# see--/speech_recognition

Measured on AMD Instinct MI355X. Metric: 1s 16kHz clips/sec training throughput, higher is better.
Workload: dtype f32; 1 GPU; configs[1]: 12-class conv_1d_time_sliced_with_attention, batch 1024/GPU synthetic 16000-sample fp32 clips, sampler+augment+STFT/mel(80,60)+raw fwd/bwd+RMSprop; global_batch=1024, parallelism=dp1, clip_bank=65536

## Files before the change

### include/kws_hip.h

```cpp
#ifndef KWS_HIP_H_
#define KWS_HIP_H_

#include <stdint.h>

#ifdef __cplusplus
extern "C" {
#endif
#if defined(__GNUC__) || defined(__clang__)
#pragma GCC visibility push(default)
#endif

#define KWS_OK 0
#define KWS_E_INVALID (-1)
#define KWS_E_HIP (-2)
#define KWS_E_WORKSPACE (-3)

#define KWS_ABI_VERSION 5

int kws_abi_version(void);
const char* kws_last_error(void);
int kws_device_name(char* buf, int cap);

int kws_stream_create(int cls, void** stream);
int kws_stream_destroy(void* stream);
// ... 72 lines not shown
int kws_comm_destroy(kws_comm_t* comm);
int kws_allreduce_grads(kws_comm_t* comm, float* grads, int64_t n, void* stream);

int kws_head32to12(const float* p_in, int C_in, const int32_t* map, int C_out, float* p_out,
                   int B, void* stream);

typedef struct kws_stft_plan kws_stft_plan_t;
int kws_stft_plan_create(int frame_len, int frame_step, int fft_len, int n_mel, int n_out,
                         const float* window, const float* mel, const float* dct,
                         float log_offset, float log_floor, kws_stft_plan_t** plan);
int kws_stft_plan_destroy(kws_stft_plan_t* plan);
int kws_stft_num_frames(const kws_stft_plan_t* plan, int L);
int kws_stft_mel_f32(const kws_stft_plan_t* plan, const float* x, int B, int L, float* out,
                     int out_kind, void* stream);

int kws_absmax_batch_f32(const float* const* in, const int64_t* n, unsigned* slots, int count, void* stream);
int kws_dwconv_fwd_amax_f32(const float* y, const float* bn, const float* w, float* z, int B, int L_in, int L_out,
                            int C, int stride, int pad_l, unsigned* amax, void* stream);
int kws_dwconv_bwd_bn_amax_f32(const float* dz, const float* y, const float* bn, const float* w, const float* coef,
                               float* dy, float* part, int pass, int B, int L_in, int L_out, int C, int stride, int pad_l,
                               unsigned* amax, void* stream);
int kws_bn_bwd_apply_amax(float* g, const float* y, const float* bn, const float* gamma, const float* coef, int64_t rows,
                          int C, unsigned* amax, void* stream);
int kws_f16x2_split_batch(const float* const* in, void* const* out, const int* rows, const int* cols,
                          const int* transpose, const unsigned* const* slots, int count, void* stream);
int kws_gemm_nn_f16x2_supported(int64_t M, int K, int N);
int kws_gemm_tn_f16x2_supported(int64_t M, int K, int N);
int kws_gemm_nn_f16x2_stats_rows(int64_t M);
int kws_gemm_nn_f16x2_f32(const float* A, const void* Bp, float* C, int64_t M, int K, int N,
                          const unsigned* a_slots, const unsigned* b_slots, float* stats_part, void* stream);
int64_t kws_gemm_tn_f16x2_workspace_floats(int64_t M, int K, int N);
int kws_gemm_tn_f16x2_f32(const float* Z, const float* G, float* dW, int64_t M, int K, int N,
                          const unsigned* z_slots, const unsigned* g_slots, float* workspace, void* stream);

int kws_gemm_num_row_tiles(int64_t M);
int kws_gemm_nn_stats_rows(int64_t M, int K, int N);
int kws_gemm_gather_stats_rows(int64_t M);
int kws_gemm_nn_f32(const float* A, const float* W, float* C, int64_t M, int K, int N,
                    float* stats_part, void* stream);
typedef struct {
  int L_out;
  int cin;
  int taps;
  int stride_t;
  int stride_j;
  int base_off;
// ... 211 lines not shown
  int kind;
  int num_classes;
  int filter_mult;
  int input_size;
  int spectrogram_length;
  int num_features;
} kws_net_config_t;
typedef struct {
  char name[64];
  int64_t offset;
  int64_t size;
  int ndim;
  int64_t shape[4];
  int is_state;
  float l2;
  int fan_in, fan_out;
  float init;
} kws_tensor_info_t;

int kws_net_create(const kws_net_config_t* cfg, kws_net_t** net);
int kws_net_destroy(kws_net_t* net);
int kws_net_get_gemm_mode(const kws_net_t* net);
int kws_net_set_gemm_mode(kws_net_t* net, int mode);
int64_t kws_net_num_params(const kws_net_t* net);
int64_t kws_net_num_state(const kws_net_t* net);
int kws_net_num_tensors(const kws_net_t* net);
int kws_net_tensor_info(const kws_net_t* net, int idx, kws_tensor_info_t* info);
int64_t kws_net_workspace_bytes(const kws_net_t* net, int max_batch, int training);
int kws_net_debug_view(const kws_net_t* net, int batch, int training, int what, int index,
                       int64_t* offset_floats, int64_t* count);
int kws_net_predict(const kws_net_t* net, const float* params, const float* state, const float* x,
                    int B, float* probs, void* workspace, int64_t workspace_bytes, void* stream);
int kws_net_train_fwd_bwd(const kws_net_t* net, const float* params, float* state, const float* x,
                          const float* y_onehot, int B, float* grads, float* probs, float* metrics,
                          uint64_t seed, uint32_t step, int64_t row_offset, int loss_batch,
                          void* workspace, int64_t workspace_bytes, void* stream);

int kws_net_num_blocks(const kws_net_t* net);
int64_t kws_net_grad_ready_offset(const kws_net_t* net, int split_block);
int kws_net_train_fwd_bwd_part(const kws_net_t* net, const float* params, float* state, const float* x,
                               const float* y_onehot, int B, float* grads, float* probs, float* metrics,
                               uint64_t seed, uint32_t step, int64_t row_offset, int loss_batch,
                               void* workspace, int64_t workspace_bytes, int part, int split_block,
                               void* stream);

#if defined(__GNUC__) || defined(__clang__)
// ... 7 lines not shown
```

### speech_recognition_amd/_lib.py

```python
import ctypes
import os

_HERE = os.path.dirname(os.path.abspath(__file__))
LIB_PATH = os.environ.get("KWS_LIB_PATH") or os.path.join(_HERE, "libkws_hip.so")

ABI_VERSION = 5

KWS_NET_TS_ATTENTION = 1
KWS_NET_LOG_MFCC = 2
KWS_NET_STEFFE = 3
KWS_NET_RESIDUAL = 4
KWS_NET_MFCC_AND_RAW = 5
KWS_NET_CONV_1D_FAST = 6
KWS_NET_CONV_1D_SPEC = 7
KWS_NET_CONV_1D_TIME_STACKED = 8
KWS_NET_CONV_1D_HEAVY = 9
KWS_NET_CONV_1D_GRU = 10
KWS_NET_CONV_1D_MULTI_TIME_SLICED = 11
KWS_NET_CONV_1D_SIMPLE = 12
KWS_NET_XCEPTION_ATTENTION = 13
KWS_NET_INCEPTION_D1 = 14
KWS_NET_CONV_2D_MOBILE = 15
KWS_NET_CONV_2D_FAST = 16
KWS_NET_CONV_1D_TIME_SLICED = 17
# ... 108 lines not shown
    "kws_allreduce_grads": (_I, [_P, _P, _I64, _P]),
    "kws_stretch_plan_create": (_I, [_I, ctypes.c_double, ctypes.POINTER(_P)]),
    "kws_stretch_plan_destroy": (_I, [_P]),
    "kws_stretch_out_samples": (_I, [_P]),
    "kws_time_stretch_f32": (_I, [_P, _P, _F, _P, _I, _I, _I, _P]),
    "kws_time_stretch_i16": (_I, [_P, _P, _P, _I, _I, _I, _P]),
    "kws_stft_plan_create": (_I, [_I, _I, _I, _I, _I, _P, _P, _P, _F, _F, ctypes.POINTER(_P)]),
    "kws_stft_plan_destroy": (_I, [_P]),
    "kws_stft_num_frames": (_I, [_P, _I]),
    "kws_stft_mel_f32": (_I, [_P, _P, _I, _I, _P, _I, _P]),
    "kws_gemm_num_row_tiles": (_I, [_I64]),
    "kws_gemm_nn_stats_rows": (_I, [_I64, _I, _I]),
    "kws_gemm_gather_stats_rows": (_I, [_I64]),
    "kws_gemm_nn_f32": (_I, [_P, _P, _P, _I64, _I, _I, _P, _P]),
    "kws_net_get_gemm_mode": (_I, [_P]),
    "kws_net_set_gemm_mode": (_I, [_P, _I]),
    "kws_gemm_nn_f16x2_supported": (_I, [_I64, _I, _I]),
    "kws_gemm_tn_f16x2_supported": (_I, [_I64, _I, _I]),
    "kws_gemm_nn_f16x2_stats_rows": (_I, [_I64]),
    "kws_absmax_batch_f32": (_I, [_P, _P, _P, _I, _P]),
    "kws_dwconv_fwd_amax_f32": (_I, [_P, _P, _P, _P, _I, _I, _I, _I, _I, _I, _P, _P]),
    "kws_dwconv_bwd_bn_amax_f32": (_I, [_P, _P, _P, _P, _P, _P, _P, _I, _I, _I, _I, _I, _I, _I, _P, _P]),
    "kws_bn_bwd_apply_amax": (_I, [_P, _P, _P, _P, _P, _I64, _I, _P, _P]),
    "kws_f16x2_split_batch": (_I, [_P, _P, _P, _P, _P, _P, _I, _P]),
    "kws_gemm_nn_f16x2_f32": (_I, [_P, _P, _P, _I64, _I, _I, _P, _P, _P, _P]),
    "kws_gemm_tn_f16x2_workspace_floats": (_I64, [_I64, _I, _I]),
    "kws_gemm_tn_f16x2_f32": (_I, [_P, _P, _P, _I64, _I, _I, _P, _P, _P, _P]),
    "kws_gemm_gather_f32": (_I, [_P, ctypes.POINTER(GatherDesc), _P, _P, _I, _I, _P, _P]),
    "kws_gemm_tn_workspace_floats": (_I64, [_I64, _I, _I]),
    "kws_gemm_tn_f32": (_I, [_P, _P, _P, _I64, _I, _I, _P, _P]),
    "kws_gemm_tn_gather_f32": (_I, [_P, ctypes.POINTER(GatherDesc), _P, _P, _I, _I, _P, _P]),
    "kws_gconv_stats_rows": (_I, [ctypes.POINTER(GconvDesc)]),
    "kws_gconv_fwd_f32": (_I, [_P, _P, _I, _P, _P, _P, ctypes.POINTER(GconvDesc), _P]),
    "kws_gconv_dgrad_f32": (_I, [_P, _P, _P, ctypes.POINTER(GconvDesc), _P]),
    "kws_gconv_wgrad_workspace_floats": (_I64, [ctypes.POINTER(GconvDesc)]),
    "kws_gconv_wgrad_f32": (_I, [_P, _P, _I, _P, _P, _P, ctypes.POINTER(GconvDesc), _P]),
    "kws_pool3s2_out_len": (_I, [_I]),
    "kws_pool3s2_fwd_f32": (_I, [_P, _P, _P, _I, _I, _I, _P]),
    "kws_pool3s2_bwd_part_rows": (_I, [_I, _I, _I]),
    "kws_pool3s2_bwd_part_floats": (_I64, [_I, _I, _I]),
    "kws_pool3s2_bwd_f32": (_I, [_P, _P, _P, _P, _P, _I, _I, _I, _P]),
    "kws_pool3s2_same_out_len": (_I, [_I]),
    "kws_pool3s2_same_fwd_f32": (_I, [_P, _P, _P, _I, _I, _I, _P]),
    "kws_pool3s2_same_bwd_part_rows": (_I, [_I, _I, _I]),
    "kws_pool3s2_same_bwd_part_floats": (_I64, [_I, _I, _I]),
    "kws_pool3s2_same_bwd_f32": (_I, [_P, _P, _P, _P, _P, _I, _I, _I, _P]),
# ... 197 lines not shown
```

### speech_recognition_amd/csrc/dw_bwd_body.h

```cpp
#pragma once
#include "internal.h"

namespace kws_dw {

#ifndef KWS_DW_NT
#define KWS_DW_NT 1
#endif
typedef float dw_v4f __attribute__((ext_vector_type(4)));
__device__ __forceinline__ float4 ld4_stream(const float* p) {
  if (KWS_DW_NT & 2) {
    const dw_v4f v = __builtin_nontemporal_load(reinterpret_cast<const dw_v4f*>(p));
    return make_float4(v.x, v.y, v.z, v.w);
  }
  return *reinterpret_cast<const float4*>(p);
}
__device__ __forceinline__ void st4_stream(float* p, float4 o) {
  if (KWS_DW_NT & 1) {
    dw_v4f v = {o.x, o.y, o.z, o.w};
    __builtin_nontemporal_store(v, reinterpret_cast<dw_v4f*>(p));
    return;
  }
  *reinterpret_cast<float4*>(p) = o;
}

// ... 2 lines not shown
#endif
constexpr int TT = KWS_DW_TT;

__device__ __forceinline__ float4 f4_fma(float4 a, float4 b, float4 c) {
  return make_float4(fmaf(a.x, b.x, c.x), fmaf(a.y, b.y, c.y), fmaf(a.z, b.z, c.z), fmaf(a.w, b.w, c.w));
}
__device__ __forceinline__ float4 f4_mul(float4 a, float4 b) {
  return make_float4(a.x * b.x, a.y * b.y, a.z * b.z, a.w * b.w);
}
__device__ __forceinline__ float4 f4_zero() { return make_float4(0.f, 0.f, 0.f, 0.f); }

#ifndef DW_BWD_THREADS
#define DW_BWD_THREADS 512
#endif
#ifndef DW_BWD_HT
#define DW_BWD_HT 8
#endif
#ifndef DW_BWD2_THREADS
#define DW_BWD2_THREADS 512
#endif
#ifndef DW_BWD_PARTS
#define DW_BWD_PARTS 256
#endif

struct BwdArgs {
  const float* dz; const float* y; const float* bn; const float* w; const float* coef;
  float* g; float* part;
  int B, Lin, Lout, C, pad_l, nchunks, R, Cb;
  unsigned* amax;
  int add_stride = 0, add_len = 0;
};
constexpr int bwd_smem_floats(int mode, int threads) { return mode == 2 ? 4 : 5 * threads * 4; }

template <int S, bool HAS_BN, int MODE, bool GUARD, bool ADDS = false>
__device__ __forceinline__ void bwd_body(const BwdArgs& p, float* const red, const int bid, const int nblk, const int by) {
  const float* __restrict__ dz = p.dz;
  const float* __restrict__ y = p.y;
  const float* __restrict__ bn = p.bn;
  const float* __restrict__ w = p.w;
  const float* __restrict__ coef = p.coef;
  float* __restrict__ g = p.g;
  float* __restrict__ part = p.part;
  const int B = p.B, Lin = p.Lin, Lout = p.Lout, C = p.C, pad_l = p.pad_l, nchunks = p.nchunks, R = p.R, Cb = p.Cb;
  constexpr int RSTRIDE = (MODE == 2 ? 4 : DW_BWD_THREADS * 4);
  float gmax = 0.f;
  const int C4 = Cb >> 2;
  const int tid = threadIdx.x;
  const bool live = !GUARD || tid < R * C4;
  const int r = live ? tid / C4 : 0, c4 = live ? tid - r * C4 : 0;
  const int c = by * Cb + c4 * 4;
  float4 sg = f4_zero(), sgx = f4_zero(), sw0 = f4_zero(), sw1 = f4_zero(), sw2 = f4_zero();
  float4 sc = f4_zero(), sh = f4_zero(), mean = f4_zero(), rstd = f4_zero();
  if (HAS_BN) {
    sc = *reinterpret_cast<const float4*>(bn + c);
    sh = *reinterpret_cast<const float4*>(bn + C + c);
    mean = *reinterpret_cast<const float4*>(bn + 2 * C + c);
    rstd = *reinterpret_cast<const float4*>(bn + 3 * C + c);
  }
  const float4 w0 = *reinterpret_cast<const float4*>(w + c);
  const float4 w1 = *reinterpret_cast<const float4*>(w + C + c);
  const float4 w2 = *reinterpret_cast<const float4*>(w + 2 * C + c);
  float4 c1 = f4_zero(), c2 = f4_zero();
  if (MODE == 2) {
    c1 = *reinterpret_cast<const float4*>(coef + c);
    c2 = *reinterpret_cast<const float4*>(coef + C + c);
  }
  for (int64_t ub = bid; ub * R < (int64_t)B * nchunks; ub += nblk) {
    const int64_t unit = ub * R + r;
    const int64_t b = unit / nchunks;
    const int chunk = (int)(unit - b * nchunks);
    if (b >= B || !live) continue;
    const float* yb = y + b * (int64_t)Lin * C + c;
    float* gb = g + b * (int64_t)Lin * C + c;
    const float* dzb = dz + b * (int64_t)Lout * C + c;
    const int u0 = chunk * TT;
    constexpr int HT = DW_BWD_HT;
    constexpr int ND = S == 1 ? HT + 2 : HT / 2 + 2;
    const bool podd = (pad_l & 1) != 0;
#pragma unroll
    for (int h = 0; h < TT / HT; ++h) {
      const int ub = u0 + h * HT;
      if (ub >= Lin) break;
      float4 yv[HT], D[ND];
#pragma unroll
      for (int i = 0; i < HT; ++i) yv[i] = ld4_stream(yb + (int64_t)(ub + i < Lin ? ub + i : ub) * C);
      const int t_lo = S == 1 ? ub + pad_l - 2 : ((ub + pad_l) >> 1) - 1;
#pragma unroll
      for (int j = 0; j < ND; ++j) {
        const int t = t_lo + j;
        D[j] = ld4_stream(dzb + (int64_t)(t < 0 ? 0 : (t < Lout ? t : Lout - 1)) * C);
      }
// ... 115 lines not shown
```

### speech_recognition_amd/csrc/dwconv.hip

```cpp
#include "dw_bwd_body.h"

namespace {
using namespace kws_dw;

#ifndef DW_FWD_GRID
#define DW_FWD_GRID 4096
#endif

template <int S, bool HAS_BN>
__global__ __launch_bounds__(256) void dwconv_fwd_kernel(const float* __restrict__ y, const float* __restrict__ bn,
                                                         const float* __restrict__ w, float* __restrict__ z,
                                                         int B, int Lin, int Lout, int C, int pad_l, int nchunks,
                                                         unsigned* amax) {
  const int C4 = C >> 2;
  float zmax = 0.f;
  const int64_t total = (int64_t)B * nchunks * C4;
  for (int64_t id = (int64_t)blockIdx.x * 256 + threadIdx.x; id < total; id += (int64_t)gridDim.x * 256) {
    const int c4 = (int)(id % C4);
    const int64_t rest = id / C4;
    const int chunk = (int)(rest % nchunks);
    const int64_t b = rest / nchunks;
    const int c = c4 * 4;
    float4 sc = f4_zero(), sh = f4_zero();
    if (HAS_BN) {
      sc = *reinterpret_cast<const float4*>(bn + c);
      sh = *reinterpret_cast<const float4*>(bn + C + c);
    }
    const float4 w0 = *reinterpret_cast<const float4*>(w + c);
    const float4 w1 = *reinterpret_cast<const float4*>(w + C + c);
    const float4 w2 = *reinterpret_cast<const float4*>(w + 2 * C + c);
    const float* yb = y + b * (int64_t)Lin * C + c;
    float* zb = z + b * (int64_t)Lout * C + c;
    constexpr int NL = S == 1 ? TT + 2 : 2 * TT + 1;
    const int t0 = chunk * TT;
    const int u_lo = S * t0 - pad_l;
    float4 av[NL];
#pragma unroll
    for (int k = 0; k < NL; ++k) {
      const int u = u_lo + k;
      av[k] = ld4_stream(yb + (int64_t)(u >= 0 && u < Lin ? u : 0) * C);
// ... 23 lines not shown
  }
  if (amax) kws_absmax_commit(amax, zmax);
}

#ifndef KWS_DW_BWD2_MINW
#define KWS_DW_BWD2_MINW 1
#endif
#ifndef KWS_DW_BWD1_MINW
#define KWS_DW_BWD1_MINW 1
#endif
template <int S, bool HAS_BN, int MODE, bool ADDS = false>
__global__ __launch_bounds__(MODE == 2 ? DW_BWD2_THREADS : DW_BWD_THREADS, MODE == 2 ? KWS_DW_BWD2_MINW : KWS_DW_BWD1_MINW) void dwconv_bwd_kernel(BwdArgs p) {
  __shared__ float red[bwd_smem_floats(MODE, DW_BWD_THREADS)];
  bwd_body<S, HAS_BN, MODE, false, ADDS>(p, red, (int)blockIdx.x, (int)gridDim.x, (int)blockIdx.y);
}

}


namespace {
template <int MODE>
int launch_dw_bwd(const float* dz, const float* y, const float* bn, const float* w, const float* coef, float* g,
                  float* part, int B, int L_in, int L_out, int C, int stride, int pad_l, hipStream_t st,
                  unsigned* amax = nullptr, int add_stride = 0, int add_len = 0) {
  const BwdGeom ge = bwd_geom(B, L_in, C, MODE != 2);
  KWS_REQUIRE(ge.grid < 0x7FFFFFFF, "dwconv_bwd: grid too large");
  dim3 gr((unsigned)ge.grid, (unsigned)ge.ny), b((unsigned)ge.block);
  BwdArgs a;
  a.dz = dz; a.y = y; a.bn = bn; a.w = w; a.coef = coef; a.g = g; a.part = part;
  a.B = B; a.Lin = L_in; a.Lout = L_out; a.C = C; a.pad_l = pad_l; a.nchunks = ge.nchunks; a.R = ge.R; a.Cb = ge.Cb; a.amax = amax;
  a.add_stride = add_stride; a.add_len = add_len;
  if (MODE == 0 && add_stride > 1) {
    if (stride == 1) hipLaunchKernelGGL((dwconv_bwd_kernel<1, false, MODE, true>), gr, b, 0, st, a);
    else hipLaunchKernelGGL((dwconv_bwd_kernel<2, false, MODE, true>), gr, b, 0, st, a);
    KWS_LAUNCH_CHECK("dwconv_bwd_kernel");
    return KWS_OK;
  }
  if (stride == 1) {
    if (bn) hipLaunchKernelGGL((dwconv_bwd_kernel<1, true, MODE>), gr, b, 0, st, a);
    else hipLaunchKernelGGL((dwconv_bwd_kernel<1, false, MODE>), gr, b, 0, st, a);
  } else {
    if (bn) hipLaunchKernelGGL((dwconv_bwd_kernel<2, true, MODE>), gr, b, 0, st, a);
    else hipLaunchKernelGGL((dwconv_bwd_kernel<2, false, MODE>), gr, b, 0, st, a);
  }
  KWS_LAUNCH_CHECK("dwconv_bwd_kernel");
  return KWS_OK;
}
}

extern "C" {

int kws_dwconv_fwd_f32(const float* y, const float* bn, const float* w, float* z, int B, int L_in, int L_out,
                       int C, int stride, int pad_l, void* stream) {
  return kws_dwconv_fwd_amax_f32(y, bn, w, z, B, L_in, L_out, C, stride, pad_l, nullptr, (hipStream_t)stream);
}

int kws_dwconv_fwd_amax_f32(const float* y, const float* bn, const float* w, float* z, int B, int L_in, int L_out,
                            int C, int stride, int pad_l, unsigned* amax, void* stream_) {
  hipStream_t stream = (hipStream_t)stream_;
  KWS_REQUIRE(y && w && z, "dwconv_fwd: NULL pointer");
  KWS_REQUIRE(B > 0 && L_in > 0 && L_out > 0 && C > 0 && C % 4 == 0, "dwconv_fwd: bad shape B=%d L=%d->%d C=%d",
              B, L_in, L_out, C);
  KWS_REQUIRE(stride == 1 || stride == 2, "dwconv_fwd: stride %d unsupported", stride);
  KWS_REQUIRE(pad_l >= 0 && stride * (L_out - 1) + 2 - pad_l < L_in + 2, "dwconv_fwd: geometry reads past padding");
  const int nchunks = ceil_div(L_out, TT);
  const int64_t threads = (int64_t)B * nchunks * (C / 4);
  int64_t grid = ceil_div64(threads, 256);
  if (grid > DW_FWD_GRID) grid = DW_FWD_GRID;
  dim3 g((unsigned)grid), b(256);
  hipStream_t st = (hipStream_t)stream;
  KwsProfScope prof("dwconv_fwd", 6.0 * B * L_out * C, 4.0 * ((double)B * L_in * C + (double)B * L_out * C), st);
  if (stride == 1) {
    if (bn) hipLaunchKernelGGL((dwconv_fwd_kernel<1, true>), g, b, 0, st, y, bn, w, z, B, L_in, L_out, C, pad_l, nchunks, amax);
    else hipLaunchKernelGGL((dwconv_fwd_kernel<1, false>), g, b, 0, st, y, bn, w, z, B, L_in, L_out, C, pad_l, nchunks, amax);
  } else {
    if (bn) hipLaunchKernelGGL((dwconv_fwd_kernel<2, true>), g, b, 0, st, y, bn, w, z, B, L_in, L_out, C, pad_l, nchunks, amax);
    else hipLaunchKernelGGL((dwconv_fwd_kernel<2, false>), g, b, 0, st, y, bn, w, z, B, L_in, L_out, C, pad_l, nchunks, amax);
  }
  KWS_LAUNCH_CHECK("dwconv_fwd_kernel");
  return KWS_OK;
}

int64_t kws_dwconv_bwd_part_floats(int B, int L_in, int C) {
  if (B <= 0 || L_in <= 0 || !bwd_geom_ok(C)) return 0;
  const BwdGeom g = bwd_geom(B, L_in, C);
  return g.grid * 5 * C;
}

int kws_dwconv_bwd_f32(const float* dz, const float* y, const float* bn, const float* w, float* g, float* part,
                       int B, int L_in, int L_out, int C, int stride, int pad_l, void* stream) {
  KWS_REQUIRE(dz && y && w && g && part, "dwconv_bwd: NULL pointer");
  KWS_REQUIRE(B > 0 && L_in > 0 && L_out > 0 && bwd_geom_ok(C),
              "dwconv_bwd: bad shape B=%d L=%d->%d C=%d", B, L_in, L_out, C);
  KWS_REQUIRE(stride == 1 || stride == 2, "dwconv_bwd: stride %d unsupported", stride);
  hipStream_t st = (hipStream_t)stream;
  KwsProfScope prof("dwconv_bwd", 12.0 * B * L_in * C, 4.0 * (2.0 * B * L_in * C + (double)B * L_out * C), st);
  return launch_dw_bwd<0>(dz, y, bn, w, nullptr, g, part, B, L_in, L_out, C, stride, pad_l, st);
}

int kws_dwconv_bwd_acc_f32(const float* dz, const float* y, const float* w, const float* add, float* g, float* part, int B,
// ... 4 lines not shown
  KwsProfScope prof("dwconv_bwd", 13.0 * B * L_in * C, 4.0 * (3.0 * B * L_in * C + (double)B * L_out * C), st);
  return launch_dw_bwd<0>(dz, y, nullptr, w, add, g, part, B, L_in, L_out, C, stride, pad_l, st);
}

int kws_dwconv_bwd_acc_strided_f32(const float* dz, const float* y, const float* w, const float* add, int add_stride, int add_len,
                                   float* g, float* part, int B, int L_in, int L_out, int C, int stride, int pad_l, hipStream_t st) {
  KWS_REQUIRE(dz && y && w && add && g && part && add != g, "dwconv_bwd_acc_strided: bad pointers");
  KWS_REQUIRE(B > 0 && L_in > 0 && L_out > 0 && bwd_geom_ok(C) && (stride == 1 || stride == 2) && add_stride >= 2 && add_len > 0 &&
                  (int64_t)(add_len - 1) * add_stride < L_in,
              "dwconv_bwd_acc_strided: bad shape B=%d L=%d->%d C=%d stride=%d add %d x %d", B, L_in, L_out, C, stride, add_len, add_stride);
  KwsProfScope prof("dwconv_bwd", 13.0 * B * L_in * C, 4.0 * (2.0 * B * L_in * C + (double)B * L_out * C + (double)B * add_len * C), st);
  return launch_dw_bwd<0>(dz, y, nullptr, w, add, g, part, B, L_in, L_out, C, stride, pad_l, st, nullptr, add_stride, add_len);
}

int kws_dwconv_bwd_bn_f32(const float* dz, const float* y, const float* bn, const float* w, const float* coef,
                          float* dy, float* part, int pass, int B, int L_in, int L_out, int C, int stride, int pad_l,
                          void* stream) {
  return kws_dwconv_bwd_bn_amax_f32(dz, y, bn, w, coef, dy, part, pass, B, L_in, L_out, C, stride, pad_l, nullptr,
                                    (hipStream_t)stream);
}

int kws_dwconv_bwd_bn_amax_f32(const float* dz, const float* y, const float* bn, const float* w, const float* coef,
                               float* dy, float* part, int pass, int B, int L_in, int L_out, int C, int stride, int pad_l,
                               unsigned* amax, void* stream_) {
  hipStream_t stream = (hipStream_t)stream_;
  KWS_REQUIRE(dz && y && bn && w, "dwconv_bwd_bn: NULL pointer");
  KWS_REQUIRE(pass == 1 ? part != nullptr : (pass == 2 && coef != nullptr && dy != nullptr),
              "dwconv_bwd_bn: pass %d needs %s", pass, pass == 1 ? "part" : "coef and dy");
  KWS_REQUIRE(B > 0 && L_in > 0 && L_out > 0 && bwd_geom_ok(C),
              "dwconv_bwd_bn: bad shape B=%d L=%d->%d C=%d", B, L_in, L_out, C);
  KWS_REQUIRE(stride == 1 || stride == 2, "dwconv_bwd_bn: stride %d unsupported", stride);
  hipStream_t st = (hipStream_t)stream;
  KwsProfScope prof("dwconv_bwd", 12.0 * B * L_in * C,
                    4.0 * ((pass == 2 ? 2.0 : 1.0) * B * L_in * C + (double)B * L_out * C), st);
  if (pass == 1) return launch_dw_bwd<1>(dz, y, bn, w, nullptr, nullptr, part, B, L_in, L_out, C, stride, pad_l, st);
  return launch_dw_bwd<2>(dz, y, bn, w, coef, dy, nullptr, B, L_in, L_out, C, stride, pad_l, st, amax);
}

}
```

### speech_recognition_amd/csrc/net.hip

```cpp
#include "net_internal.h"
#include <math.h>
#include <stdlib.h>

int64_t kws_net_add_tensor(kws_net* n, const std::string& name, std::vector<int64_t> shape, bool is_state, float l2,
                           int fan_in, int fan_out, float init) {
  kws_tensor_info_t t;
  memset(&t, 0, sizeof(t));
  snprintf(t.name, sizeof(t.name), "%s", name.c_str());
  int64_t size = 1;
  t.ndim = (int)shape.size();
  for (int i = 0; i < t.ndim; ++i) {
    t.shape[i] = shape[i];
    size *= shape[i];
  }
  t.size = size;
  t.is_state = is_state ? 1 : 0;
  t.l2 = l2;
  t.fan_in = fan_in;
  t.fan_out = fan_out;
  t.init = init;
  int64_t& cursor = is_state ? n->n_state : n->n_params;
  t.offset = cursor;
  cursor += (size + 3) / 4 * 4;
  n->tensors.push_back(t);
// ... 485 lines not shown
}

int kws_net_debug_view(const kws_net_t* net, int batch, int training, int what, int index, int64_t* offset_floats,
                       int64_t* count) {
  KWS_REQUIRE(net && offset_floats && count && batch > 0, "net_debug_view: bad arguments");
  return net->program->debug_view(batch, training, what, index, offset_floats, count);
}

int kws_net_predict(const kws_net_t* net, const float* params, const float* state, const float* x, int B,
                    float* probs, void* workspace, int64_t workspace_bytes, void* stream) {
  KWS_REQUIRE(net && params && state && x && probs && workspace && B > 0, "net_predict: bad arguments");
  return net->program->predict(params, state, x, B, probs, (float*)workspace, workspace_bytes, (hipStream_t)stream);
}

extern "C" int kws_net_get_gemm_mode(const kws_net_t* net) { return net ? net->gemm_mode.load(std::memory_order_relaxed) : 0; }
extern "C" int kws_net_set_gemm_mode(kws_net_t* net, int mode) {
  KWS_REQUIRE(net != nullptr, "net_set_gemm_mode: NULL net");
  KWS_REQUIRE(mode >= 0 && mode <= 2,
              "net_set_gemm_mode: mode %d (0 = f32 MFMA, 1 = f32 MFMA with separate input- / weight-gradient launches, 2 = fp16 x 2 split)", mode);
  net->gemm_mode.store(mode, std::memory_order_relaxed);
  return KWS_OK;
}

int kws_net_train_fwd_bwd(const kws_net_t* net, const float* params, float* state, const float* x,
                          const float* y_onehot, int B, float* grads, float* probs, float* metrics, uint64_t seed,
                          uint32_t step, int64_t row_offset, int loss_batch, void* workspace, int64_t workspace_bytes,
                          void* stream) {
  KWS_REQUIRE(net && params && state && x && y_onehot && grads && probs && metrics && workspace && B > 0,
              "net_train_fwd_bwd: bad arguments");
  KWS_REQUIRE(loss_batch >= B, "net_train_fwd_bwd: loss_batch %d < B %d", loss_batch, B);
  return net->program->train(params, state, x, y_onehot, B, grads, probs, metrics, seed, step, row_offset, loss_batch, (float*)workspace,
                             workspace_bytes, (hipStream_t)stream);
}

static const TsProgram* ts_program(const kws_net_t* net) {
  return (net && net->cfg.kind == KWS_NET_TS_ATTENTION) ? static_cast<const TsProgram*>(net->program.get()) : nullptr;
}

int kws_net_num_blocks(const kws_net_t* net) {
  const TsProgram* ts = ts_program(net);
  return ts ? ts->lad.nb() : 0;
}

int64_t kws_net_grad_ready_offset(const kws_net_t* net, int split_block) {
  const TsProgram* ts = ts_program(net);
  if (!ts || split_block < 1 || split_block >= ts->lad.nb()) return -1;
// ... 20 lines not shown
```

### speech_recognition_amd/csrc/net_dw3ladder.hip

```cpp
#include "net_internal.h"

int Dw3Ladder::build(KerasNames& kn, const int (*spec)[2], int n, int fm, int input_size) {
  int L = L1, cin = C1;
  for (int i = 0; i < n; ++i) {
    Dw3Block b;
    b.stride = spec[i][0];
    b.cin = cin;
    b.cout = spec[i][1] * fm;
    b.Lin = L;
    if (b.stride == 2) {
      kws_same_pad(L, 3, 2, &b.Lout, &b.pad_l);
    } else {
      b.Lout = L - 2;
      b.pad_l = 0;
    }
    KWS_REQUIRE(b.Lout >= 1, "net: input_size %d is too short: block %d keeps no row", input_size, i);
    b.dw = kn.dw(cin);
    b.pw = kn.conv(1, cin, b.cout, KWS_L2_COEF);
    b.bn = kn.bn(b.cout);
    blocks.push_back(b);
    L = b.Lout;
    cin = b.cout;
  }
  return KWS_OK;
}

// ... 62 lines not shown
  KWS_REQUIRE(nb() + 1 <= KWS_BN_INFER_BATCH, "net: %d blocks exceed the BatchNorm table batch", nb());
  const float *ga[KWS_BN_INFER_BATCH], *be[KWS_BN_INFER_BATCH], *mm[KWS_BN_INFER_BATCH], *mv[KWS_BN_INFER_BATCH];
  float* tb[KWS_BN_INFER_BATCH];
  int Cs[KWS_BN_INFER_BATCH];
  for (int l = 0; l <= nb(); ++l) {
    const BnRef& b = l == 0 ? bn1 : blocks[l - 1].bn;
    ga[l] = r.params + b.gamma; be[l] = r.params + b.beta; mm[l] = r.state + b.mm; mv[l] = r.state + b.mv; tb[l] = r.bn_at(l); Cs[l] = b.C;
  }
  return kws_bn_infer_prepare_batch(ga, be, mm, mv, KWS_BN_EPS, Cs, tb, nb() + 1, r.st);
}

int Dw3Ladder::transpose_all(const Dw3Run& r) const {
  KWS_REQUIRE(nb() <= KWS_TRANSPOSE_BATCH, "net: %d blocks exceed the transpose batch", nb());
  const float* tin[KWS_TRANSPOSE_BATCH];
  float* tout[KWS_TRANSPOSE_BATCH];
  int trows[KWS_TRANSPOSE_BATCH], tcols[KWS_TRANSPOSE_BATCH];
  for (int i = 0; i < nb(); ++i) {
    tin[i] = r.params + blocks[i].pw; tout[i] = r.WT(i);
    trows[i] = blocks[i].cin; tcols[i] = blocks[i].cout;
  }
  return kws_transpose_batch_f32(tin, tout, trows, tcols, nb(), r.st);
}

int Dw3Ladder::fwd_dw(int i, const Dw3Run& r, unsigned* amax) const {
  const Dw3Block& b = blocks[i];
  return kws_dwconv_fwd_amax_f32(r.y(i), r.bn_at(i), r.params + b.dw, r.z(i), r.B, b.Lin, b.Lout, b.cin, b.stride, b.pad_l, amax, r.st);
}

int Dw3Ladder::stats_finalize(int i, const Dw3Run& r, const float* stats, int rows) const {
  const Dw3Block& b = blocks[i];
  return kws_bn_stats_finalize(stats, rows, (int64_t)r.B * b.Lout, b.cout, r.params + b.bn.gamma, r.params + b.bn.beta, KWS_BN_EPS,
                               KWS_BN_MOMENTUM, r.state + b.bn.mm, r.state + b.bn.mv, r.bn_at(i + 1), r.red, r.st);
}

int Dw3Ladder::fwd_block_f32(int i, const Dw3Run& r, float* stats, unsigned* amax) const {
  const Dw3Block& b = blocks[i];
  const int64_t M = (int64_t)r.B * b.Lout;
  KWS_TRY(fwd_dw(i, r, amax));
  KWS_TRY(kws_gemm_nn_f32(r.z(i), r.params + b.pw, r.y(i + 1), M, b.cin, b.cout, stats, r.st));
  return stats ? stats_finalize(i, r, stats, kws_gemm_nn_stats_rows(M, b.cin, b.cout)) : KWS_OK;
}

int Dw3Ladder::bwd_block_input(int i, const Dw3Run& r, float* dy, unsigned* amax) const {
  const Dw3Block& b = blocks[i];
  const BnRef& prev = (i == 0) ? bn1 : blocks[i - 1].bn;
  KWS_TRY(kws_dwconv_bwd_bn_f32(r.DZ, r.y(i), r.bn_at(i), r.params + b.dw, nullptr, nullptr, r.part, 1, r.B, b.Lin, b.Lout, b.cin,
                                b.stride, b.pad_l, r.st));
  const int n_parts = (int)(kws_dwconv_bwd_part_floats(r.B, b.Lin, b.cin) / (5 * b.cin));
  KWS_TRY(kws_dw_bwd_finalize(r.part, n_parts, (int64_t)r.B * b.Lin, b.cin, r.grads + b.dw, r.grads + prev.gamma, r.grads + prev.beta,
                              r.coef, r.red, r.st));
  return kws_dwconv_bwd_bn_amax_f32(r.DZ, r.y(i), r.bn_at(i), r.params + b.dw, r.coef, dy, nullptr, 2, r.B, b.Lin, b.Lout, b.cin, b.stride,
                                    b.pad_l, amax, r.st);
}
```

### speech_recognition_amd/csrc/net_internal.h

```cpp
#pragma once
#include <string.h>

#include <algorithm>
#include <atomic>
#include <memory>
#include <string>
#include <vector>

#include "internal.h"

constexpr float KWS_BN_EPS = 1e-3f;
constexpr float KWS_BN_MOMENTUM = 0.99f;
constexpr float KWS_L2_COEF = 1e-5f;

struct BnRef {
  int64_t gamma, beta;
  int64_t mm, mv;
  int C;
};
inline kws_gbn_refs kws_gbn_layer_refs(const BnRef& r, const float* params, float* state) {
  return kws_gbn_refs{params + r.gamma, 0, r.beta - r.gamma, state + r.mm, 0, r.mv - r.mm};
}
inline int kws_gbn_layer_bwd(float* dA, const float* y, const float* bn, const float* add, int64_t M, const kws_gbn_cols& c, float* part,
                             float* coef, float* grads, const BnRef& r, hipStream_t st) {
// ... 1 lines not shown
}
inline int kws_gbn_layer_bwd_finish(float* g, const float* y, const float* bn, int64_t M, const kws_gbn_cols& c, const float* part, int rows,
                                    float* coef, float* grads, const BnRef& r, hipStream_t st) {
  return kws_gbn_bwd_finish(g, y, bn, M, &c, part, rows, coef, grads + r.gamma, 0, r.beta - r.gamma, st);
}

struct NetProgram {
  virtual ~NetProgram() {}
  virtual int64_t workspace_bytes(int B, int training) const = 0;
  virtual int debug_view(int B, int training, int what, int index, int64_t* offset_floats, int64_t* count) const = 0;
  virtual int predict(const float* params, const float* state, const float* x, int B, float* probs, float* ws, int64_t ws_bytes,
                      hipStream_t st) const = 0;
  virtual int train(const float* params, float* state, const float* x, const float* y_onehot, int B, float* grads, float* probs,
                    float* metrics, uint64_t seed, uint32_t step, int64_t row_offset, int loss_batch, float* ws, int64_t ws_bytes,
                    hipStream_t st) const = 0;
};

struct kws_net {
  kws_net_config_t cfg;
  std::vector<kws_tensor_info_t> tensors;
  int64_t n_params = 0, n_state = 0;
  std::unique_ptr<NetProgram> program;
  std::atomic<int> gemm_mode{0};
};

int64_t kws_net_add_tensor(kws_net* n, const std::string& name, std::vector<int64_t> shape, bool is_state, float l2,
                           int fan_in, int fan_out, float init);
BnRef kws_net_add_bn(kws_net* n, int idx, int C);
void kws_same_pad(int L, int k, int s, int* Lout, int* pl);

struct KerasNames {
  kws_net* n;
  int n_conv = 0, n_bn = 0, n_dw = 0;
  int64_t conv(int k, int cin, int cout, float l2);
  BnRef bn(int C, int* idx = nullptr);
  int64_t dw(int C);
  int64_t dwk(int k, int C);
};

struct Bump {
  int64_t cur = 0;
  int64_t take(int64_t floats) {
    const int64_t o = cur;
    cur += (floats + 63) / 64 * 64;
    return o;
  }
};
// ... 50 lines not shown
struct Dw3Offsets {
  std::vector<int64_t> y, z;
  std::vector<int64_t> WT;
  int64_t bn = 0, bn_stride = 0;
};
struct Dw3Run {
  const Dw3Offsets* o;
  const float* params;
  float* state;
  float* grads;
  float* ws;
  int B;
  float *red, *part, *coef, *DZ;
  hipStream_t st;
  float* y(int l) const { return ws + o->y[l]; }
  float* z(int i) const { return ws + o->z[i]; }
  float* WT(int i) const { return ws + o->WT[i]; }
  float* bn_at(int l) const { return ws + o->bn + o->bn_stride * l; }
};
struct Dw3Ladder {
  int L1 = 0, C1 = 0;
  BnRef bn1;
  std::vector<Dw3Block> blocks;
  int nb() const { return (int)blocks.size(); }
  int build(KerasNames& kn, const int (*spec)[2], int n, int fm, int input_size);
  Dw3Sizes sizes(int B) const;
  void take_acts(Bump& bp, int B, bool training, const Dw3Sizes& s, Dw3Offsets* o) const;
  void take_bn(Bump& bp, int maxC, Dw3Offsets* o) const;
  void take_WT(Bump& bp, Dw3Offsets* o) const;
  int debug_view(const Dw3Offsets& o, int B, int what, int index, int64_t* offset_floats, int64_t* count) const;
  int infer_tables(const Dw3Run& r) const;
  int transpose_all(const Dw3Run& r) const;
  int fwd_dw(int i, const Dw3Run& r, unsigned* amax) const;
  int stats_finalize(int i, const Dw3Run& r, const float* stats, int rows) const;
  int fwd_block_f32(int i, const Dw3Run& r, float* stats, unsigned* amax) const;
  int bwd_block_input(int i, const Dw3Run& r, float* dy, unsigned* amax) const;
};

int kws_block_out_fwd(const float* y, const float* bn, const float* res, const float* res_bn, float* o, int B,
                      int L, int C, int pool, hipStream_t st);
int kws_block_out_dw_fwd(const float* y, const float* bn, const float* res, const float* res_bn, const float* w, float* o, float* z, int B,
                         int L, int C, int pool, hipStream_t st);
int kws_block_join_bwd_parts(int B, int L, int C, int pool);
int kws_block_join_bwd(const float* dO, const float* y, const float* bn, const float* gamma, const float* coef, float* out,
                       float* part, int pass, int B, int L, int C, int pool, int relu, hipStream_t st);
int64_t kws_block_out_bwd_part_floats(int B, int L, int C, int pool);
int kws_block_out_bwd(const float* dO, const float* y, const float* bn, float* g, float* part, int B, int L, int C,
// ... 49 lines not shown
```

### speech_recognition_amd/net.py

```python
import ctypes
from collections import OrderedDict

import numpy as np
import torch

from . import _lib
from ._lib import KWS_NET_LOG_MFCC, KWS_NET_TS_ATTENTION


class TensorSpec(object):
    __slots__ = ("name", "offset", "size", "shape", "is_state", "l2", "fan_in", "fan_out", "init")

    def __repr__(self):
        return "TensorSpec(%s %s @%d)" % (self.name, self.shape, self.offset)


class DeviceNet(object):

    def __init__(self, kind, num_classes, filter_mult=1, input_size=16000, spectrogram_length=0,
                 num_features=0, device=None, seed=87654321, gemm_mode=None):
        if not torch.cuda.is_available():
            raise _lib.KwsError("no MI355X visible to this process: the HIP path is the only path "
                                "(no CPU fallback)")
        self.lib = _lib.load()
# ... 14 lines not shown
            _lib.check(self.lib.kws_net_tensor_info(h, i, ctypes.byref(ti)), "kws_net_tensor_info")
            s = TensorSpec()
            s.name = ti.name.decode()
            s.offset, s.size = int(ti.offset), int(ti.size)
            s.shape = tuple(int(ti.shape[k]) for k in range(ti.ndim))
            s.is_state = bool(ti.is_state)
            s.l2, s.fan_in, s.fan_out, s.init = float(ti.l2), ti.fan_in, ti.fan_out, float(ti.init)
            self.tensors[s.name] = s
        with torch.cuda.device(self.device):
            self.params = torch.zeros(self.n_params, dtype=torch.float32, device=self.device)
            self.state = torch.zeros(self.n_state, dtype=torch.float32, device=self.device)
            self.grads = torch.zeros(self.n_params, dtype=torch.float32, device=self.device)
            self.slots = torch.zeros(self.n_params, dtype=torch.float32, device=self.device)
            self.l2 = torch.zeros(self.n_params, dtype=torch.float32, device=self.device)
            self.metrics = torch.zeros(4, dtype=torch.float32, device=self.device)
            self.reg_loss = torch.zeros(1, dtype=torch.float32, device=self.device)
        self.slots2 = None
        self._ws = None
        self._ws_key = None
        if gemm_mode is None:
            import os
            gemm_mode = 2 if os.environ.get("KWS_GEMM_F16X2") else 0
        self.set_gemm_mode(gemm_mode)
        self.initialize(seed)

    @property
    def gemm_mode(self):
        return int(self.lib.kws_net_get_gemm_mode(self.handle))

    def set_gemm_mode(self, mode):
        _lib.check(self.lib.kws_net_set_gemm_mode(self.handle, int(mode)), "kws_net_set_gemm_mode")

    def __del__(self):
        try:
            if getattr(self, "handle", None):
                self.lib.kws_net_destroy(self.handle)
                self.handle = None
        except Exception:
            pass

    def count_params(self):
        return sum(s.size for s in self.tensors.values())

    def trainable_count(self):
        return sum(s.size for s in self.tensors.values() if not s.is_state)

    def initialize(self, seed=87654321):
        rng = np.random.RandomState(seed)
        n_orth = 0
        p = np.zeros(self.n_params, np.float32)
        st = np.zeros(self.n_state, np.float32)
        l2 = np.zeros(self.n_params, np.float32)
        for s in self.tensors.values():
            dst = st if s.is_state else p
# ... 128 lines not shown
```

Measured before the change: 232,700 clips/s.

## Sweep depthwise conv kernels in descending order to reuse cache-resident producer data

Adds a descending traversal option to the depthwise conv forward and backward pass-2 kernels. Work is walked in reverse granules so the consumer first touches the tail of the tensor the producer wrote last, which is more likely still in L2 or MALL. A per-block planner compares modeled residency for same-direction and opposite-direction sweeps against assumed L2/MALL capacities and picks one. Granule alignment keeps amax slot assignment per wave, at the cost of padded grids and a few idle threads.

```diff
diff --git a/include/kws_hip.h b/include/kws_hip.h
--- a/include/kws_hip.h
+++ b/include/kws_hip.h
@@ -118,6 +118,12 @@
                                unsigned* amax, void* stream);
 int kws_bn_bwd_apply_amax(float* g, const float* y, const float* bn, const float* gamma, const float* coef, int64_t rows,
                           int C, unsigned* amax, void* stream);
+int kws_dwconv_fwd_dir_f32(const float* y, const float* bn, const float* w, float* z, int B, int L_in, int L_out,
+                           int C, int stride, int pad_l, unsigned* amax, int descending, void* stream);
+int kws_dwconv_bwd_bn_dir_f32(const float* dz, const float* y, const float* bn, const float* w, const float* coef,
+                              float* dy, float* part, int pass, int B, int L_in, int L_out, int C, int stride, int pad_l,
+                              unsigned* amax, int descending, void* stream);
+int kws_sweep_descending(int64_t producer_bytes, int64_t consumer_bytes, int64_t capacity_bytes);
 int kws_f16x2_split_batch(const float* const* in, void* const* out, const int* rows, const int* cols,
                           const int* transpose, const unsigned* const* slots, int count, void* stream);
 int kws_gemm_nn_f16x2_supported(int64_t M, int K, int N);
@@ -375,6 +381,8 @@
 int kws_net_destroy(kws_net_t* net);
 int kws_net_get_gemm_mode(const kws_net_t* net);
 int kws_net_set_gemm_mode(kws_net_t* net, int mode);
+int kws_net_get_sweep_mode(const kws_net_t* net);
+int kws_net_set_sweep_mode(kws_net_t* net, int mode);
 int64_t kws_net_num_params(const kws_net_t* net);
 int64_t kws_net_num_state(const kws_net_t* net);
 int kws_net_num_tensors(const kws_net_t* net);
diff --git a/speech_recognition_amd/_lib.py b/speech_recognition_amd/_lib.py
--- a/speech_recognition_amd/_lib.py
+++ b/speech_recognition_amd/_lib.py
@@ -154,6 +154,11 @@
     "kws_dwconv_fwd_amax_f32": (_I, [_P, _P, _P, _P, _I, _I, _I, _I, _I, _I, _P, _P]),
     "kws_dwconv_bwd_bn_amax_f32": (_I, [_P, _P, _P, _P, _P, _P, _P, _I, _I, _I, _I, _I, _I, _I, _P, _P]),
     "kws_bn_bwd_apply_amax": (_I, [_P, _P, _P, _P, _P, _I64, _I, _P, _P]),
+    "kws_dwconv_fwd_dir_f32": (_I, [_P, _P, _P, _P, _I, _I, _I, _I, _I, _I, _P, _I, _P]),
+    "kws_dwconv_bwd_bn_dir_f32": (_I, [_P, _P, _P, _P, _P, _P, _P, _I, _I, _I, _I, _I, _I, _I, _P, _I, _P]),
+    "kws_sweep_descending": (_I, [_I64, _I64, _I64]),
+    "kws_net_get_sweep_mode": (_I, [_P]),
+    "kws_net_set_sweep_mode": (_I, [_P, _I]),
     "kws_f16x2_split_batch": (_I, [_P, _P, _P, _P, _P, _P, _I, _P]),
     "kws_gemm_nn_f16x2_f32": (_I, [_P, _P, _P, _I64, _I, _I, _P, _P, _P, _P]),
     "kws_gemm_tn_f16x2_workspace_floats": (_I64, [_I64, _I, _I]),
diff --git a/speech_recognition_amd/csrc/dw_bwd_body.h b/speech_recognition_amd/csrc/dw_bwd_body.h
--- a/speech_recognition_amd/csrc/dw_bwd_body.h
+++ b/speech_recognition_amd/csrc/dw_bwd_body.h
@@ -48,6 +48,8 @@
 #ifndef DW_BWD_PARTS
 #define DW_BWD_PARTS 256
 #endif
+
+constexpr int DW_BWD_GRANULE = KWS_ABSMAX_SLOTS;
 
 struct BwdArgs {
   const float* dz; const float* y; const float* bn; const float* w; const float* coef;
@@ -55,6 +57,7 @@
   int B, Lin, Lout, C, pad_l, nchunks, R, Cb;
   unsigned* amax;
   int add_stride = 0, add_len = 0;
+  int descending = 0;
 };
 constexpr int bwd_smem_floats(int mode, int threads) { return mode == 2 ? 4 : 5 * threads * 4; }
 
@@ -91,8 +94,11 @@
     c1 = *reinterpret_cast<const float4*>(coef + c);
     c2 = *reinterpret_cast<const float4*>(coef + C + c);
   }
-  for (int64_t ub = bid; ub * R < (int64_t)B * nchunks; ub += nblk) {
-    const int64_t unit = ub * R + r;
+  const int64_t gspan = MODE == 2 && p.descending
+                            ? (((int64_t)B * nchunks + R - 1) / R + DW_BWD_GRANULE - 1) / DW_BWD_GRANULE * DW_BWD_GRANULE : 0;
+  for (int64_t ub = bid; MODE == 2 && gspan ? ub < gspan : ub * R < (int64_t)B * nchunks; ub += nblk) {
+    const int64_t unit =
+        (MODE == 2 && gspan ? gspan - DW_BWD_GRANULE - (ub & ~(int64_t)(DW_BWD_GRANULE - 1)) + (ub & (DW_BWD_GRANULE - 1)) : ub) * R + r;
     const int64_t b = unit / nchunks;
     const int chunk = (int)(unit - b * nchunks);
     if (b >= B || !live) continue;
diff --git a/speech_recognition_amd/csrc/dwconv.hip b/speech_recognition_amd/csrc/dwconv.hip
--- a/speech_recognition_amd/csrc/dwconv.hip
+++ b/speech_recognition_amd/csrc/dwconv.hip
@@ -6,16 +6,24 @@
 #ifndef DW_FWD_GRID
 #define DW_FWD_GRID 4096
 #endif
+constexpr int DW_FWD_GRANULE = 64 * KWS_ABSMAX_SLOTS;
+static_assert(DW_FWD_GRID % (DW_FWD_GRANULE / 256) == 0, "a grid-stride trip must keep a wave's amax slot");
 
 template <int S, bool HAS_BN>
 __global__ __launch_bounds__(256) void dwconv_fwd_kernel(const float* __restrict__ y, const float* __restrict__ bn,
                                                          const float* __restrict__ w, float* __restrict__ z,
                                                          int B, int Lin, int Lout, int C, int pad_l, int nchunks,
-                                                         unsigned* amax) {
+                                                         unsigned* amax, int descending) {
   const int C4 = C >> 2;
   float zmax = 0.f;
   const int64_t total = (int64_t)B * nchunks * C4;
-  for (int64_t id = (int64_t)blockIdx.x * 256 + threadIdx.x; id < total; id += (int64_t)gridDim.x * 256) {
+  const int64_t span = descending ? (total + DW_FWD_GRANULE - 1) / DW_FWD_GRANULE * DW_FWD_GRANULE : total;
+  for (int64_t gid = (int64_t)blockIdx.x * 256 + threadIdx.x; gid < span; gid += (int64_t)gridDim.x * 256) {
+    int64_t id = gid;
+    if (descending) {
+      id = span - DW_FWD_GRANULE - (gid & ~(int64_t)(DW_FWD_GRANULE - 1)) + (gid & (DW_FWD_GRANULE - 1));
+      if (id >= total) continue;
+    }
     const int c4 = (int)(id % C4);
     const int64_t rest = id / C4;
     const int chunk = (int)(rest % nchunks);
@@ -85,14 +93,16 @@
 template <int MODE>
 int launch_dw_bwd(const float* dz, const float* y, const float* bn, const float* w, const float* coef, float* g,
                   float* part, int B, int L_in, int L_out, int C, int stride, int pad_l, hipStream_t st,
-                  unsigned* amax = nullptr, int add_stride = 0, int add_len = 0) {
-  const BwdGeom ge = bwd_geom(B, L_in, C, MODE != 2);
+                  unsigned* amax = nullptr, int add_stride = 0, int add_len = 0, int descending = 0) {
+  KWS_REQUIRE(MODE == 2 || !descending, "dwconv_bwd: only pass 2 sweeps descending (the sums of the other modes are order-bound)");
+  BwdGeom ge = bwd_geom(B, L_in, C, MODE != 2);
+  if (descending) ge.grid = std::min<int64_t>((ge.grid + DW_BWD_GRANULE - 1) / DW_BWD_GRANULE * DW_BWD_GRANULE, 1024);
   KWS_REQUIRE(ge.grid < 0x7FFFFFFF, "dwconv_bwd: grid too large");
   dim3 gr((unsigned)ge.grid, (unsigned)ge.ny), b((unsigned)ge.block);
   BwdArgs a;
   a.dz = dz; a.y = y; a.bn = bn; a.w = w; a.coef = coef; a.g = g; a.part = part;
   a.B = B; a.Lin = L_in; a.Lout = L_out; a.C = C; a.pad_l = pad_l; a.nchunks = ge.nchunks; a.R = ge.R; a.Cb = ge.Cb; a.amax = amax;
-  a.add_stride = add_stride; a.add_len = add_len;
+  a.add_stride = add_stride; a.add_len = add_len; a.descending = descending;
   if (MODE == 0 && add_stride > 1) {
     if (stride == 1) hipLaunchKernelGGL((dwconv_bwd_kernel<1, false, MODE, true>), gr, b, 0, st, a);
     else hipLaunchKernelGGL((dwconv_bwd_kernel<2, false, MODE, true>), gr, b, 0, st, a);
@@ -119,8 +129,14 @@
 }
 
 int kws_dwconv_fwd_amax_f32(const float* y, const float* bn, const float* w, float* z, int B, int L_in, int L_out,
-                            int C, int stride, int pad_l, unsigned* amax, void* stream_) {
+                            int C, int stride, int pad_l, unsigned* amax, void* stream) {
+  return kws_dwconv_fwd_dir_f32(y, bn, w, z, B, L_in, L_out, C, stride, pad_l, amax, 0, stream);
+}
+
+int kws_dwconv_fwd_dir_f32(const float* y, const float* bn, const float* w, float* z, int B, int L_in, int L_out,
+                           int C, int stride, int pad_l, unsigned* amax, int descending, void* stream_) {
   hipStream_t stream = (hipStream_t)stream_;
+  descending = descending != 0;
   KWS_REQUIRE(y && w && z, "dwconv_fwd: NULL pointer");
   KWS_REQUIRE(B > 0 && L_in > 0 && L_out > 0 && C > 0 && C % 4 == 0, "dwconv_fwd: bad shape B=%d L=%d->%d C=%d",
               B, L_in, L_out, C);
@@ -129,16 +145,17 @@
   const int nchunks = ceil_div(L_out, TT);
   const int64_t threads = (int64_t)B * nchunks * (C / 4);
   int64_t grid = ceil_div64(threads, 256);
+  if (descending) grid = ceil_div64(threads, DW_FWD_GRANULE) * (DW_FWD_GRANULE / 256);
   if (grid > DW_FWD_GRID) grid = DW_FWD_GRID;
   dim3 g((unsigned)grid), b(256);
   hipStream_t st = (hipStream_t)stream;
   KwsProfScope prof("dwconv_fwd", 6.0 * B * L_out * C, 4.0 * ((double)B * L_in * C + (double)B * L_out * C), st);
   if (stride == 1) {
-    if (bn) hipLaunchKernelGGL((dwconv_fwd_kernel<1, true>), g, b, 0, st, y, bn, w, z, B, L_in, L_out, C, pad_l, nchunks, amax);
-    else hipLaunchKernelGGL((dwconv_fwd_kernel<1, false>), g, b, 0, st, y, bn, w, z, B, L_in, L_out, C, pad_l, nchunks, amax);
+    if (bn) hipLaunchKernelGGL((dwconv_fwd_kernel<1, true>), g, b, 0, st, y, bn, w, z, B, L_in, L_out, C, pad_l, nchunks, amax, descending);
+    else hipLaunchKernelGGL((dwconv_fwd_kernel<1, false>), g, b, 0, st, y, bn, w, z, B, L_in, L_out, C, pad_l, nchunks, amax, descending);
   } else {
-    if (bn) hipLaunchKernelGGL((dwconv_fwd_kernel<2, true>), g, b, 0, st, y, bn, w, z, B, L_in, L_out, C, pad_l, nchunks, amax);
-    else hipLaunchKernelGGL((dwconv_fwd_kernel<2, false>), g, b, 0, st, y, bn, w, z, B, L_in, L_out, C, pad_l, nchunks, amax);
+    if (bn) hipLaunchKernelGGL((dwconv_fwd_kernel<2, true>), g, b, 0, st, y, bn, w, z, B, L_in, L_out, C, pad_l, nchunks, amax, descending);
+    else hipLaunchKernelGGL((dwconv_fwd_kernel<2, false>), g, b, 0, st, y, bn, w, z, B, L_in, L_out, C, pad_l, nchunks, amax, descending);
   }
   KWS_LAUNCH_CHECK("dwconv_fwd_kernel");
   return KWS_OK;
@@ -189,8 +206,15 @@
 
 int kws_dwconv_bwd_bn_amax_f32(const float* dz, const float* y, const float* bn, const float* w, const float* coef,
                                float* dy, float* part, int pass, int B, int L_in, int L_out, int C, int stride, int pad_l,
-                               unsigned* amax, void* stream_) {
+                               unsigned* amax, void* stream) {
+  return kws_dwconv_bwd_bn_dir_f32(dz, y, bn, w, coef, dy, part, pass, B, L_in, L_out, C, stride, pad_l, amax, 0, stream);
+}
+
+int kws_dwconv_bwd_bn_dir_f32(const float* dz, const float* y, const float* bn, const float* w, const float* coef,
+                              float* dy, float* part, int pass, int B, int L_in, int L_out, int C, int stride, int pad_l,
+                              unsigned* amax, int descending, void* stream_) {
   hipStream_t stream = (hipStream_t)stream_;
+  KWS_REQUIRE(pass == 2 || !descending, "dwconv_bwd_bn: pass %d cannot sweep descending (its sums are order-bound)", pass);
   KWS_REQUIRE(dz && y && bn && w, "dwconv_bwd_bn: NULL pointer");
   KWS_REQUIRE(pass == 1 ? part != nullptr : (pass == 2 && coef != nullptr && dy != nullptr),
               "dwconv_bwd_bn: pass %d needs %s", pass, pass == 1 ? "part" : "coef and dy");
@@ -201,7 +225,7 @@
   KwsProfScope prof("dwconv_bwd", 12.0 * B * L_in * C,
                     4.0 * ((pass == 2 ? 2.0 : 1.0) * B * L_in * C + (double)B * L_out * C), st);
   if (pass == 1) return launch_dw_bwd<1>(dz, y, bn, w, nullptr, nullptr, part, B, L_in, L_out, C, stride, pad_l, st);
-  return launch_dw_bwd<2>(dz, y, bn, w, coef, dy, nullptr, B, L_in, L_out, C, stride, pad_l, st, amax);
-}
-
-}
+  return launch_dw_bwd<2>(dz, y, bn, w, coef, dy, nullptr, B, L_in, L_out, C, stride, pad_l, st, amax, 0, 0, descending != 0);
+}
+
+}
diff --git a/speech_recognition_amd/csrc/net.hip b/speech_recognition_amd/csrc/net.hip
--- a/speech_recognition_amd/csrc/net.hip
+++ b/speech_recognition_amd/csrc/net.hip
@@ -531,6 +531,14 @@
   return KWS_OK;
 }
 
+extern "C" int kws_net_get_sweep_mode(const kws_net_t* net) { return net ? net->sweep_mode.load(std::memory_order_relaxed) : 0; }
+extern "C" int kws_net_set_sweep_mode(kws_net_t* net, int mode) {
+  KWS_REQUIRE(net != nullptr, "net_set_sweep_mode: NULL net");
+  KWS_REQUIRE(mode >= 0 && mode <= 2, "net_set_sweep_mode: mode %d (0 = planned per block, 1 = all ascending, 2 = all descending)", mode);
+  net->sweep_mode.store(mode, std::memory_order_relaxed);
+  return KWS_OK;
+}
+
 int kws_net_train_fwd_bwd(const kws_net_t* net, const float* params, float* state, const float* x,
                           const float* y_onehot, int B, float* grads, float* probs, float* metrics, uint64_t seed,
                           uint32_t step, int64_t row_offset, int loss_batch, void* workspace, int64_t workspace_bytes,
diff --git a/speech_recognition_amd/csrc/net_dw3ladder.hip b/speech_recognition_amd/csrc/net_dw3ladder.hip
--- a/speech_recognition_amd/csrc/net_dw3ladder.hip
+++ b/speech_recognition_amd/csrc/net_dw3ladder.hip
@@ -2,6 +2,8 @@
 
 int Dw3Ladder::build(KerasNames& kn, const int (*spec)[2], int n, int fm, int input_size) {
   int L = L1, cin = C1;
+  net = kn.n;
+  clip_floats = input_size;
   for (int i = 0; i < n; ++i) {
     Dw3Block b;
     b.stride = spec[i][0];
@@ -110,9 +112,27 @@
   return kws_transpose_batch_f32(tin, tout, trows, tcols, nb(), r.st);
 }
 
+int Dw3Ladder::fwd_descending(int i, int B) const {
+  const int mode = kws_net_get_sweep_mode(net);
+  if (mode != 0) return mode == 2;
+  const Dw3Block& b = blocks[i];
+  const int64_t y = (int64_t)B * b.Lin * b.cin * 4, z = (int64_t)B * b.Lout * b.cin * 4;
+  const int64_t a = i == 0 ? (int64_t)B * clip_floats * 4 : (int64_t)B * blocks[i - 1].Lout * blocks[i - 1].cin * 4;
+  return kws_sweep_plan(a + y, y + z, KWS_SWEEP_MALL_BYTES);
+}
+
+int Dw3Ladder::bwd2_descending(int i, int B) const {
+  const int mode = kws_net_get_sweep_mode(net);
+  if (mode != 0) return mode == 2;
+  const Dw3Block& b = blocks[i];
+  const int64_t y = (int64_t)B * b.Lin * b.cin * 4, dz = (int64_t)B * b.Lout * b.cin * 4;
+  return kws_sweep_plan(dz + y, dz + y + y, KWS_SWEEP_L2_BYTES);
+}
+
 int Dw3Ladder::fwd_dw(int i, const Dw3Run& r, unsigned* amax) const {
   const Dw3Block& b = blocks[i];
-  return kws_dwconv_fwd_amax_f32(r.y(i), r.bn_at(i), r.params + b.dw, r.z(i), r.B, b.Lin, b.Lout, b.cin, b.stride, b.pad_l, amax, r.st);
+  return kws_dwconv_fwd_dir_f32(r.y(i), r.bn_at(i), r.params + b.dw, r.z(i), r.B, b.Lin, b.Lout, b.cin, b.stride, b.pad_l, amax,
+                                fwd_descending(i, r.B), r.st);
 }
 
 int Dw3Ladder::stats_finalize(int i, const Dw3Run& r, const float* stats, int rows) const {
@@ -137,6 +157,10 @@
   const int n_parts = (int)(kws_dwconv_bwd_part_floats(r.B, b.Lin, b.cin) / (5 * b.cin));
   KWS_TRY(kws_dw_bwd_finalize(r.part, n_parts, (int64_t)r.B * b.Lin, b.cin, r.grads + b.dw, r.grads + prev.gamma, r.grads + prev.beta,
                               r.coef, r.red, r.st));
-  return kws_dwconv_bwd_bn_amax_f32(r.DZ, r.y(i), r.bn_at(i), r.params + b.dw, r.coef, dy, nullptr, 2, r.B, b.Lin, b.Lout, b.cin, b.stride,
-                                    b.pad_l, amax, r.st);
+  return kws_dwconv_bwd_bn_dir_f32(r.DZ, r.y(i), r.bn_at(i), r.params + b.dw, r.coef, dy, nullptr, 2, r.B, b.Lin, b.Lout, b.cin, b.stride,
+                                   b.pad_l, amax, bwd2_descending(i, r.B), r.st);
 }
+
+extern "C" int kws_sweep_descending(int64_t producer_bytes, int64_t consumer_bytes, int64_t capacity_bytes) {
+  return kws_sweep_plan(producer_bytes, consumer_bytes, capacity_bytes);
+}
diff --git a/speech_recognition_amd/csrc/net_internal.h b/speech_recognition_amd/csrc/net_internal.h
--- a/speech_recognition_amd/csrc/net_internal.h
+++ b/speech_recognition_amd/csrc/net_internal.h
@@ -47,7 +47,24 @@
   int64_t n_params = 0, n_state = 0;
   std::unique_ptr<NetProgram> program;
   std::atomic<int> gemm_mode{0};
-};
+  std::atomic<int> sweep_mode{0};
+};
+
+constexpr int64_t KWS_SWEEP_MALL_BYTES = (int64_t)256 << 20;
+constexpr int64_t KWS_SWEEP_L2_BYTES = (int64_t)8 * (4 << 20);
+inline double kws_sweep_resident_same(int64_t p, int64_t q, int64_t cap) {
+  if (p <= cap && q <= cap) return 1.0;
+  if (q <= cap) return (double)(cap - q) / (double)(p - q);
+  if (p <= cap) return (double)(cap - p) / (double)(q - p);
+  return 0.0;
+}
+inline double kws_sweep_resident_opposite(int64_t p, int64_t q, int64_t cap) {
+  return p + q <= cap ? 1.0 : (double)cap / (double)(p + q);
+}
+inline int kws_sweep_plan(int64_t p, int64_t q, int64_t cap) {
+  if (p <= 0 || q <= 0 || cap <= 0) return 0;
+  return kws_sweep_resident_opposite(p, q, cap) > kws_sweep_resident_same(p, q, cap) ? 1 : 0;
+}
 
 int64_t kws_net_add_tensor(kws_net* n, const std::string& name, std::vector<int64_t> shape, bool is_state, float l2,
                            int fan_in, int fan_out, float init);
@@ -144,7 +161,11 @@
   int L1 = 0, C1 = 0;
   BnRef bn1;
   std::vector<Dw3Block> blocks;
+  const kws_net* net = nullptr;
+  int clip_floats = 0;
   int nb() const { return (int)blocks.size(); }
+  int fwd_descending(int i, int B) const;
+  int bwd2_descending(int i, int B) const;
   int build(KerasNames& kn, const int (*spec)[2], int n, int fm, int input_size);
   Dw3Sizes sizes(int B) const;
   void take_acts(Bump& bp, int B, bool training, const Dw3Sizes& s, Dw3Offsets* o) const;
diff --git a/speech_recognition_amd/net.py b/speech_recognition_amd/net.py
--- a/speech_recognition_amd/net.py
+++ b/speech_recognition_amd/net.py
@@ -60,6 +60,9 @@
             import os
             gemm_mode = 2 if os.environ.get("KWS_GEMM_F16X2") else 0
         self.set_gemm_mode(gemm_mode)
+        import os
+        if os.environ.get("KWS_SWEEP_MODE"):
+            self.set_sweep_mode(int(os.environ["KWS_SWEEP_MODE"]))
         self.initialize(seed)
 
     @property
@@ -68,6 +71,13 @@
 
     def set_gemm_mode(self, mode):
         _lib.check(self.lib.kws_net_set_gemm_mode(self.handle, int(mode)), "kws_net_set_gemm_mode")
+
+    @property
+    def sweep_mode(self):
+        return int(self.lib.kws_net_get_sweep_mode(self.handle))
+
+    def set_sweep_mode(self, mode):
+        _lib.check(self.lib.kws_net_set_sweep_mode(self.handle, int(mode)), "kws_net_set_sweep_mode")
 
     def __del__(self):
         try:
```

Result: no change. 234,200 clips/s, median of 6 (+0.6%).
